# facebookresearch/co-tracker

Hardware: NVIDIA H100
Metric: tracked points*frames/sec at N=6400, T=16, 512^2 (higher is better)
Workload: dtype transformer + corr_mlp.fc2 + input_transform: bf16x3; correlation einsum: fp16x2; corr_mlp.fc1: bf16x3; fp32 accumulate, fp32 softmax/LayerNorm/GELU

## Files before the change

cotracker_b200/csrc/api_loop.cu:

```cuda
#include <math.h>

#include <string>
#include <vector>

#include "abi.cuh"

using namespace ct3;

namespace {

struct Block {
  Lin qkv_h;
  Lin q;
  Lin kv;
  Lin out, fc1, fc2;
  size_t ctx_g = 0, ctx_b = 0;
  bool cross = false;
};
struct Layout {
  Lin corr_fc1, corr_fc2, in_tr;
  Lin corr_fc1_h;
  Lin corr_fc1_t, corr_fc1_th;
  Block time[kDepth], vself[kDepth], p2v[kDepth], v2p[kDepth];
  size_t heads_w = 0, heads_b = 0, virt = 0, win_f32 = 0;
  size_t total = 0;
};

void place_block(Block& b, bool cross, size_t& off, bool time = false) {
  b.cross = cross;
  if (time) place_lin(b.qkv_h, 3 * kC, kC, off);
  if (cross) {
    b.ctx_g = off; off = align_up(off + kC * sizeof(float));
    b.ctx_b = off; off = align_up(off + kC * sizeof(float));
    place_lin(b.q, kC, kC, off);
    place_lin(b.kv, 2 * kC, kC, off);
  } else {
    place_lin(b.q, 3 * kC, kC, off);
  }
  place_lin(b.out, kC, kC, off);
  place_lin(b.fc1, kMlpHid, kC, off);
  place_lin(b.fc2, kC, kMlpHid, off);
}
const Layout& layout() {
  static const Layout L0 = [] {
    Layout L;
    size_t off = 0;
    place_lin(L.corr_fc1, kCorrHid, kVol, off);
    place_lin(L.corr_fc1_h, kCorrHid, kVol, off);
    place_lin(L.corr_fc1_t, kCorrHid, kVol, off);
    place_lin(L.corr_fc1_th, kCorrHid, kVol, off);
    place_lin(L.corr_fc2, kCorrOut, kCorrHid, off);
    place_lin(L.in_tr, kC, kX, off);
    L.win_f32 = off; off = align_up(off + (size_t)kC * kX * sizeof(float));
    L.virt = off;    off = align_up(off + (size_t)kV * kC * sizeof(float));
    L.heads_w = off; off = align_up(off + 4 * kC * sizeof(float));
    L.heads_b = off; off = align_up(off + 4 * sizeof(float));
    for (int i = 0; i < kDepth; ++i) {
      place_block(L.time[i], false, off,  true);
      place_block(L.vself[i], false, off);
      place_block(L.p2v[i], true, off);
      place_block(L.v2p[i], true, off);
    }
    L.total = off;
    return L;
  }();
  return L0;
}

const std::vector<std::string>& weight_names() {
  static const std::vector<std::string> names0 = [] {
    std::vector<std::string> names;
    const char* head[] = {"corr_mlp.fc1.weight", "corr_mlp.fc1.bias", "corr_mlp.fc2.weight", "corr_mlp.fc2.bias",
                          "updateformer.input_transform.weight", "updateformer.input_transform.bias",
                          "updateformer.virual_tracks", "updateformer.flow_head.weight", "updateformer.flow_head.bias",
                          "updateformer.vis_conf_head.weight", "updateformer.vis_conf_head.bias"};
    for (const char* h : head) names.push_back(h);
    const char* self_t[] = {"attn.to_q.weight", "attn.to_q.bias", "attn.to_kv.weight", "attn.to_kv.bias",
                            "attn.to_out.weight", "attn.to_out.bias", "mlp.fc1.weight", "mlp.fc1.bias",
                            "mlp.fc2.weight", "mlp.fc2.bias"};
    const char* cross_t[] = {"norm_context.weight", "norm_context.bias", "cross_attn.to_q.weight",
                             "cross_attn.to_q.bias", "cross_attn.to_kv.weight", "cross_attn.to_kv.bias",
                             "cross_attn.to_out.weight", "cross_attn.to_out.bias", "mlp.fc1.weight", "mlp.fc1.bias",
                             "mlp.fc2.weight", "mlp.fc2.bias"};
    for (int i = 0; i < kDepth; ++i) {
      const std::string idx = std::to_string(i) + ".";
      for (const char* t : self_t) names.push_back("updateformer.time_blocks." + idx + t);
      for (const char* t : self_t) names.push_back("updateformer.space_virtual_blocks." + idx + t);
      for (const char* t : cross_t) names.push_back("updateformer.space_point2virtual_blocks." + idx + t);
      for (const char* t : cross_t) names.push_back("updateformer.space_virtual2point_blocks." + idx + t);
    }
    return names;
  }();
  return names0;
}

struct Workspace {
  __nv_bfloat16* vol;
  __nv_bfloat16* h1;
  __nv_bfloat16* xs;
  float* tokens;
  __nv_bfloat16* ln;
  __nv_bfloat16* att;
  float* qkv;
  float* vqkv;
  __nv_bfloat16* hmid;
  float* row_bias;
  float* att_part;
  __nv_bfloat16* pyr_split;
  int32_t* groups;
  int32_t* frames;
  int32_t* track_len;
  int32_t* track_group;
  int slab;
  size_t total;
  bool slabbed() const { return slab_rows < point_rows; }
  int64_t slab_rows = 0, point_rows = 0;
};
int partial_slots(int N, int G) {
  if (G == 1) return kAttnMaxSplits;
  const int64_t s = kAttnMaxSplits + ((int64_t)N + 63LL * G) / 128;
  return (int)(s < (int64_t)kAttnMaxSplits * G ? s : (int64_t)kAttnMaxSplits * G);
}
int64_t group_table_ints(int N, int G) { return (int64_t)5 * G + 1 + 2 * ((int64_t)N / 128 + G); }
bool grouped(const ct3_loop_shape& s) { return s.G > 1 || s.group_T; }

Workspace carve(void* base, const ct3_loop_shape& s) {
  Workspace w;
  const int T = s.T, N = s.N, G = s.G, H4 = s.H4, W4 = s.W4, T_pyr = s.T_pyr > 0 ? s.T_pyr : s.T;
  w.slab = s.slab_tracks > 0 && s.slab_tracks < N ? s.slab_tracks : N;
  const size_t R = (size_t)(N + (size_t)kV * G) * T, Rp = (size_t)N * T, Rv = (size_t)kV * G * T;
  const size_t S = (size_t)w.slab * T, Mc = S * kL;
  w.slab_rows = (int64_t)S;
  w.point_rows = (int64_t)Rp;
  const bool sl = w.slabbed();
  Carver c(base);
  w.vol = (__nv_bfloat16*)c.take(Mc * 2 * kVolPad * 2);
  w.h1 = (__nv_bfloat16*)c.take(Mc * 2 * kCorrHid * 2);
  w.xs = (__nv_bfloat16*)c.take(S * 2 * kXPad * 2);
  w.tokens = (float*)c.take(R * kC * 4);
  w.ln = (__nv_bfloat16*)c.take((S + Rv) * 2 * kC * 2);
  w.att = (__nv_bfloat16*)c.take((S + Rv) * 2 * kC * 2);
  w.qkv = (float*)c.take(sl ? (S * 3 > Rp * 2 ? S * 3 : Rp * 2) * kC * 4 : R * 3 * kC * 4);
  w.vqkv = (float*)c.take(Rv * 3 * kC * 4);
  w.hmid = (__nv_bfloat16*)c.take((sl ? S : R) * 2 * kMlpHid * 2);
  w.row_bias = (float*)c.take((size_t)(s.group_T ? G : 1) * T * kC * 4);
  w.att_part = (float*)c.take(attention_partial_bytes(T, kV, partial_slots(N, G)));
  w.pyr_split = nullptr;
  if (H4 > 0 && W4 > 0 && corr_patch_supported(T_pyr, H4, W4))
    w.pyr_split = (__nv_bfloat16*)c.take((size_t)pyramid_layout(T_pyr, H4, W4).total * 4);
  w.groups = grouped(s) ? (int32_t*)c.take((size_t)group_table_ints(N, G) * 4) : nullptr;
  w.frames = s.T_pyr > 0 ? (int32_t*)c.take((size_t)G * T * 4) : nullptr;
  w.track_len = s.group_T ? (int32_t*)c.take(((size_t)N + (size_t)kV * G) * 4) : nullptr;
  w.track_group = s.group_T ? (int32_t*)c.take((size_t)N * 4) : nullptr;
  w.total = c.off;
  return w;
}

struct Runner {
  const uint8_t* pk;
  const Layout& L;
  cudaStream_t s;
  int impl;

  int gemm(const char* what, const __nv_bfloat16* x, const Lin& lin, int M, const GemmEpilogue& e, int products = 3,
           int fp16 = 0, int64_t x_ld = 0) {
    GemmProblem p;
    p.products = products;
    p.fp16 = fp16;
    p.x_ld = x_ld;
    p.x_split = x;
    p.w_split = reinterpret_cast<const __nv_bfloat16*>(pk + lin.w);
    p.M = M;
    p.N = lin.N;
    p.Kpad = lin.Kpad;
    p.epi = e;
    if (!p.epi.bias) p.epi.bias = reinterpret_cast<const float*>(pk + lin.b);
    if (M == 0) return 0;
    ProfScope ps(s, CAT_GEMM, 2.0 * (double)M * lin.N * lin.K);
    return run_gemm(p, impl, s, what);
  }
  static GemmEpilogue to_f32(float* out, int ld, bool residual) {
    GemmEpilogue e;
    e.out_f32 = out; e.ld_f32 = ld; e.residual = residual ? 1 : 0;
    return e;
  }
  static GemmEpilogue to_split(__nv_bfloat16* out, int ld, int lo_off, int act) {
    GemmEpilogue e;
    e.out_split = out; e.ld_split = ld; e.lo_off = lo_off; e.act = act;
    return e;
  }
};

#define RUNC(cat, call)                                        \
  do {                                                         \
    cudaError_t e__;                                           \
    { ProfScope ps__(R.s, cat); e__ = (cudaError_t)(call); }   \
    if (e__ != cudaSuccess) return fail_cuda(e__, #call);      \
  } while (0)
#define GEMM(...)                                                              \
  do {                                                                         \
    if (int rc__ = R.gemm("gemm(" #__VA_ARGS__ ")", __VA_ARGS__)) return rc__; \
  } while (0)

int run_attention(Runner& R, const Workspace& W, const AttnParams& a, bool per_warp) {
  if (g_opt_attn == 1) return (int)launch_attention(a, R.s);
  if (!per_warp && a.Lq > kV && attention_p2v_supported(a)) return (int)launch_attention_p2v(a, R.s);
  return (int)launch_attention_tc(a, per_warp, W.att_part, num_sms(), R.s);
}

AttnParams attn_params(const float* q, int q_ld, const float* kv, int kv_ld, int k_col, int v_col, __nv_bfloat16* out,
                       int Lq, int Lk, int T, int tracks = 0) {
  AttnParams a{};
  a.q = q; a.q_ld = q_ld; a.q_col = 0;
  a.kv = kv; a.kv_ld = kv_ld; a.k_col = k_col; a.v_col = v_col;
  a.out = out; a.out_ld = 2 * kC; a.lo_off = kC;
  a.num_seq = tracks ? tracks : T; a.Lq = Lq; a.Lk = Lk;
  a.q_seq_stride = a.k_seq_stride = tracks ? T : 1;
  a.q_tok_stride = a.k_tok_stride = tracks ? 1 : T;
  a.scale = 1.0f / sqrtf((float)kDh);
  return a;
}

struct GroupPlan {
  int G = 1, max_n = 0;
  const int32_t *off = nullptr, *all = nullptr, *split = nullptr, *slot = nullptr, *small = nullptr, *tile = nullptr;
  int n_small = 0, n_tiles = 0, split_max = 1, split_slots = 0;
  const int32_t *track_len = nullptr, *track_len_host = nullptr;
};

int plan_groups(GroupPlan& gp, const int32_t* sizes, int G, int T, int N, const int32_t* group_T, int32_t* dev,
                cudaStream_t s) {
  gp.G = G;
  if (G == 1 && !group_T) return 0;
  std::vector<int32_t> h((size_t)group_table_ints(N, G), 0);
  int32_t* off = h.data();
  int32_t *all = off + G + 1, *split = all + G, *slot = split + G, *small = slot + G, *tile = small + G;
  const int nsm = num_sms();
  for (int g = 0; g < G; ++g) {
    const int n = sizes ? sizes[g] : N;
    off[g + 1] = off[g] + n;
    if (n > gp.max_n) gp.max_n = n;
    all[g] = g;
    split[g] = attention_tc_splits(group_T ? group_T[g] : T, kV, n, nsm);
    if (split[g] > 1) {
      slot[g] = gp.split_slots;
      gp.split_slots += split[g];
      if (split[g] > gp.split_max) gp.split_max = split[g];
    }
    if (n > kV) {
      for (int n0 = off[g]; n0 < off[g + 1]; n0 += 128, ++gp.n_tiles) {
        tile[2 * gp.n_tiles] = g;
        tile[2 * gp.n_tiles + 1] = n0;
      }
    } else {
      small[gp.n_small++] = g;
    }
  }
  if (gp.split_slots > partial_slots(N, G)) return fail(CT3_EINVAL, "split-K partials exceed the workspace%s");
  CK(launch_upload_i32(dev, h.data(), (int)h.size(), s), "upload group table");
  gp.off = dev;
  gp.all = dev + (all - off);
  gp.split = dev + (split - off);
  gp.slot = dev + (slot - off);
  gp.small = dev + (small - off);
  gp.tile = dev + (tile - off);
  return 0;
}

int space_attention(Runner& R, const Workspace& W, const GroupPlan& gp, AttnParams a, bool q_pts, bool k_pts) {
  if (!gp.off) return run_attention(R, W, a, false);
  const int T = a.num_seq, n_all = a.Lq;
  a.goff = gp.off;
  a.frames = T;
  a.q_grp_stride = q_pts ? 0 : (int64_t)kV * a.q_tok_stride;
  a.k_grp_stride = k_pts ? 0 : (int64_t)kV * a.k_tok_stride;
  a.Lq = q_pts ? gp.max_n : kV;
  a.Lk = k_pts ? gp.max_n : kV;
  AttnParams b = a;
  b.gl = gp.all;
  b.num_seq = T * gp.G;
  if (g_opt_attn == 1) return (int)launch_attention(b, R.s);
  if (!q_pts) {
    if (k_pts) { b.gsplit = gp.split; b.gslot = gp.slot; b.split_max = gp.split_max; b.split_slots = gp.split_slots; }
    return (int)launch_attention_tc(b, false, W.att_part, num_sms(), R.s);
  }
  if (gp.n_small > 0) {
    b.gl = gp.small;
    b.num_seq = T * gp.n_small;
    b.Lq = kV;
    if (int rc = (int)launch_attention_tc(b, false, W.att_part, num_sms(), R.s)) return rc;
  }
  if (gp.n_tiles > 0) {
    AttnParams c = a;
    c.gtile = gp.tile;
    c.tiles = gp.n_tiles;
    c.Lq = n_all;
    c.Lk = kV * gp.G;
    return (int)launch_attention_p2v(c, R.s);
  }
  return 0;
}

int time_attention(Runner& R, const Workspace& W, const Block& b, const __nv_bfloat16* x, __nv_bfloat16* att,
                   int rows, int T, const int32_t* len = nullptr, const int32_t* len_host = nullptr) {
  const bool fuse = g_opt[OPT_FUSE] == 1 && R.impl == 0 && g_opt_attn != 1;
  auto fused = [&](int track0, int tracks) -> int {
    ProfScope ps(R.s, CAT_QKVA, 0.0);
    const char* gerr = nullptr;
    const int64_t r0 = (int64_t)track0 * T;
    const int rc = gemm_qkv_time_attn_launch(
        x + r0 * 2 * kC, reinterpret_cast<const __nv_bfloat16*>(R.pk + b.qkv_h.w),
        reinterpret_cast<const float*>(R.pk + b.qkv_h.b), tracks * T, kC, T, len ? len + track0 : nullptr,
        att + r0 * 2 * kC, 2 * kC, kC, 1.0f / sqrtf((float)kDh), num_sms(), R.s, &gerr);
    return rc ? fail_launch(rc, "fused qkv + time attention", gerr) : 0;
  };
  auto unfused = [&](int track0, int tracks) -> int {
    const int64_t r0 = (int64_t)track0 * T;
    GEMM(x + r0 * 2 * kC, b.q, tracks * T, Runner::to_f32(W.qkv, 3 * kC, false));
    AttnParams a = attn_params(W.qkv, 3 * kC, W.qkv, 3 * kC, kC, 2 * kC, att + r0 * 2 * kC, T, T, T, tracks);
    a.seq_len = len ? len + track0 : nullptr;
    RUNC(CAT_ATTN, run_attention(R, W, a, true));
    return 0;
  };
  if (fuse && qkv_time_attn_supported(T)) return fused(0, rows / T);
  if (!fuse || !len_host) return unfused(0, rows / T);
  for (int i = 0, n = rows / T; i < n;) {
    const bool short_run = qkv_time_attn_supported(len_host[i]);
    int j = i + 1;
    while (j < n && qkv_time_attn_supported(len_host[j]) == short_run) ++j;
    if (short_run) {
      if (int rc = fused(i, j - i)) return rc;
      const size_t row_bytes = 2 * kC * sizeof(__nv_bfloat16);
      CK(cudaMemset2DAsync(att + ((int64_t)i * T + 128) * 2 * kC, (size_t)T * row_bytes, 0,
                           (size_t)(T - 128) * row_bytes, (size_t)(j - i), R.s),
         "zero padded time-attention rows");
    } else if (int rc = unfused(i, j - i)) {
      return rc;
    }
    i = j;
  }
  return 0;
}

int64_t scratch_row(const Workspace& W, int64_t row, int64_t slab_row0) { return W.slabbed() ? row - slab_row0 : row; }

template <class F>
int for_slabs(const Workspace& W, int N, int n_begin, int n_end, F&& f) {
  if (!W.slabbed()) return f(n_begin, n_end - n_begin);
  for (int n = n_begin; n < n_end;) {
    const int stop = n < N && n_end > N ? N : n_end;
    const int count = stop - n < W.slab ? stop - n : W.slab;
    if (int rc = f(n, count)) return rc;
    n += count;
  }
  return 0;
}

int mlp_half(Runner& R, const Workspace& W, const Block& b, int64_t row0, int rows, int64_t slab_row0) {
  float* x = W.tokens + row0 * kC;
  const int64_t s = scratch_row(W, row0, slab_row0);
  __nv_bfloat16* ln = W.ln + s * 2 * kC;
  __nv_bfloat16* hm = W.hmid + s * 2 * kMlpHid;
  RUNC(CAT_LN, launch_layernorm_split(x, rows, nullptr, nullptr, 1e-6f, ln, R.s));
  GEMM(ln, b.fc1, rows, Runner::to_split(hm, 2 * kMlpHid, kMlpHid,  2));
  GEMM(hm, b.fc2, rows, Runner::to_f32(x, kC, true));
  return 0;
}

int transformer_body(Runner& R, const Workspace& W, int T, int N, const GroupPlan& gp) {
  const Layout& L = R.L;
  const int NV = kV * gp.G, Rp = N * T, Rv = NV * T;
  const uint8_t* pk = R.pk;
  RUNC(CAT_MISC, launch_init_virtual(W.tokens, reinterpret_cast<const float*>(pk + L.virt), T, N, gp.G, R.s));
  float* vtok = W.tokens + (int64_t)Rp * kC;
  __nv_bfloat16* ln_v = W.ln + W.slab_rows * 2 * kC;
  __nv_bfloat16* att_v = W.att + W.slab_rows * 2 * kC;
  float* q_p = W.qkv;
  __nv_bfloat16* att_p = W.slabbed() ? reinterpret_cast<__nv_bfloat16*>(W.qkv + (int64_t)Rp * kC) : W.att;
  auto ln_gemm_points = [&](const Block& b, bool ctx, const Lin& lin, float* out, int ld) {
    return for_slabs(W, N, 0, N, [&](int n, int count) -> int {
      const int64_t r0 = (int64_t)n * T;
      __nv_bfloat16* ln = W.ln + scratch_row(W, r0, r0) * 2 * kC;
      RUNC(CAT_LN, launch_layernorm_split(W.tokens + r0 * kC, count * T,
                                          ctx ? reinterpret_cast<const float*>(pk + b.ctx_g) : nullptr,
                                          ctx ? reinterpret_cast<const float*>(pk + b.ctx_b) : nullptr,
                                          ctx ? 1e-5f : 1e-6f, ln, R.s));
      GEMM(ln, lin, count * T, Runner::to_f32(out + r0 * ld, ld, false));
      return 0;
    });
  };
  auto mlp_tracks = [&](const Block& b, int n_begin, int n_end) {
    return for_slabs(W, N, n_begin, n_end, [&](int n, int count) -> int {
      return mlp_half(R, W, b, (int64_t)n * T, count * T, (int64_t)n * T);
    });
  };

  for (int i = 0; i < kDepth; ++i) {
    {
      const Block& b = L.time[i];
      if (int rc = for_slabs(W, N, 0, N + NV, [&](int n, int count) -> int {
            const int64_t r0 = (int64_t)n * T;
            const int rows = count * T;
            const int64_t s0 = scratch_row(W, r0, r0);
            float* x = W.tokens + r0 * kC;
            RUNC(CAT_LN, launch_layernorm_split(x, rows, nullptr, nullptr, 1e-6f, W.ln + s0 * 2 * kC, R.s));
            if (int rc = time_attention(R, W, b, W.ln + s0 * 2 * kC, W.att + s0 * 2 * kC, rows, T,
                                        gp.track_len ? gp.track_len + n : nullptr,
                                        gp.track_len_host ? gp.track_len_host + n : nullptr))
              return rc;
            GEMM(W.att + s0 * 2 * kC, b.out, rows, Runner::to_f32(x, kC, true));
            return mlp_half(R, W, b, r0, rows, r0);
          }))
        return rc;
    }
    {
      const Block& b = L.v2p[i];
      RUNC(CAT_LN, launch_layernorm_split(vtok, Rv, nullptr, nullptr, 1e-6f, ln_v, R.s));
      GEMM(ln_v, b.q, Rv, Runner::to_f32(W.vqkv, kC, false));
      if (int rc = ln_gemm_points(b, true, b.kv, W.qkv, 2 * kC)) return rc;
      RUNC(CAT_ATTN, space_attention(R, W, gp, attn_params(W.vqkv, kC, W.qkv, 2 * kC, 0, kC, att_v, kV, N, T), false,
                                     true));
      GEMM(att_v, b.out, Rv, Runner::to_f32(vtok, kC, true));
      if (int rc = mlp_tracks(b, N, N + NV)) return rc;
    }
    {
      const Block& b = L.vself[i];
      RUNC(CAT_LN, launch_layernorm_split(vtok, Rv, nullptr, nullptr, 1e-6f, ln_v, R.s));
      GEMM(ln_v, b.q, Rv, Runner::to_f32(W.vqkv, 3 * kC, false));
      RUNC(CAT_ATTN, space_attention(R, W, gp, attn_params(W.vqkv, 3 * kC, W.vqkv, 3 * kC, kC, 2 * kC, att_v, kV, kV,
                                                           T), false, false));
      GEMM(att_v, b.out, Rv, Runner::to_f32(vtok, kC, true));
      if (int rc = mlp_tracks(b, N, N + NV)) return rc;
    }
    {
      const Block& b = L.p2v[i];
      if (int rc = ln_gemm_points(b, false, b.q, q_p, kC)) return rc;
      RUNC(CAT_LN, launch_layernorm_split(vtok, Rv, reinterpret_cast<const float*>(pk + b.ctx_g),
                                 reinterpret_cast<const float*>(pk + b.ctx_b), 1e-5f, ln_v, R.s));
      GEMM(ln_v, b.kv, Rv, Runner::to_f32(W.vqkv, 2 * kC, false));
      RUNC(CAT_ATTN, space_attention(R, W, gp, attn_params(q_p, kC, W.vqkv, 2 * kC, 0, kC, att_p, N, kV, T), true,
                                     false));
      if (int rc = for_slabs(W, N, 0, N, [&](int n, int count) -> int {
            const int64_t r0 = (int64_t)n * T;
            GEMM(att_p + r0 * 2 * kC, b.out, count * T, Runner::to_f32(W.tokens + r0 * kC, kC, true));
            return mlp_half(R, W, b, r0, count * T, r0);
          }))
        return rc;
    }
  }
  return 0;
}

struct Prec {
  int corr, fc1; bool patch;
  bool vol16() const { return fc1 < 3; }
  bool support_major() const { return patch && corr != 3; }
};
Prec effective_prec(bool have_pyr_split, int T, int H4, int W4) {
  Prec p;
  p.patch = corr_uses_patch_kernel(g_opt_corr, have_pyr_split, T, H4, W4);
  p.corr = p.patch ? g_opt[OPT_PREC_CORR] : 3;
  p.fc1 = p.patch ? g_opt[OPT_PREC_FC1] : 3;
  return p;
}

int input_transform(Runner& R, const Workspace& W, int T, int n0, int count, const float* row_bias) {
  GemmEpilogue e = Runner::to_f32(W.tokens + (int64_t)n0 * T * kC, kC, false);
  if (row_bias) { e.row_bias = row_bias; e.row_mod = T; }
  if (row_bias && W.track_group) e.row_blk = W.track_group + n0;
  GEMM(W.xs, R.L.in_tr, count * T, e);
  return 0;
}

int point_tokens_slab(Runner& R, const Workspace& W, const Prec& pr, const float* pyr, const __nv_bfloat16* pyr_split,
                      int H4, int W4, const float* support, const uint8_t* track_valid, const float* coords,
                      const float* vis, const float* conf, int T, int N, int T_pyr, const FrameMap& fm, int n0,
                      int count) {
  const Layout& L = R.L;
  const int Mc = count * T * kL;
  RUNC(CAT_CORR, launch_corr_sample(pyr, pyr_split, H4, W4, support, track_valid, coords, T, N, n0, count, W.vol,
                                    g_opt_corr, pr.corr, pr.vol16() ? 1 : 0, num_sms(), R.s, T_pyr, fm));
  if (pr.vol16()) {
    GEMM(W.vol, pr.support_major() ? L.corr_fc1_th : L.corr_fc1_h, Mc,
         Runner::to_split(W.h1, 2 * kCorrHid, kCorrHid,  1), pr.fc1,  1, kVolPad);
  } else {
    GEMM(W.vol, pr.support_major() ? L.corr_fc1_t : L.corr_fc1, Mc,
         Runner::to_split(W.h1, 2 * kCorrHid, kCorrHid,  1));
  }
  {
    GemmEpilogue e = Runner::to_split(W.xs, 2 * kXPad, kXPad, 0);
    e.row_group = kL;
    GEMM(W.h1, L.corr_fc2, Mc, e);
  }
  RUNC(CAT_MISC, launch_build_x_small(coords, vis, conf, T, N, n0, count, W.track_len, W.xs, R.s));
  return input_transform(R, W, T, n0, count, W.row_bias);
}

int point_tokens(Runner& R, const Workspace& W, const Prec& pr, const float* pyr, const __nv_bfloat16* pyr_split,
                 int H4, int W4, const float* support, const uint8_t* track_valid, const float* coords,
                 const float* vis, const float* conf, int T, int N, int T_pyr, const FrameMap& fm) {
  return for_slabs(W, N, 0, N, [&](int n0, int count) -> int {
    return point_tokens_slab(R, W, pr, pyr, pyr_split, H4, W4, support, track_valid, coords, vis, conf, T, N, T_pyr,
                             fm, n0, count);
  });
}


int transform_and_heads(Runner& R, const Workspace& W, int T, int N, const GroupPlan& gp, float* coords, float* vis,
                        float* conf, float* delta) {
  const Layout& L = R.L;
  if (int rc = transformer_body(R, W, T, N, gp)) return rc;
  RUNC(CAT_MISC, launch_heads(W.tokens, reinterpret_cast<const float*>(R.pk + L.heads_w),
                              reinterpret_cast<const float*>(R.pk + L.heads_b), coords, vis, conf, delta, T, N, R.s));
  return 0;
}

int check_TN(int T, int N, int G = 1) {
  if (T < 1 || N < 1) return fail(CT3_EINVAL, "T and N must be >= 1%s");
  if (G < 1 || G > N) return fail(CT3_EINVAL, "G must be in [1, N]%s");
  if (((int64_t)N + (int64_t)kV * G) * T * 3 * kC >= (int64_t)1 << 40) return fail(CT3_EINVAL, "problem too large%s");
  return 0;
}

constexpr int64_t kSlabbedMaxRows = (int64_t)1 << 21;

enum class Use { kSize, kLoop, kFormer };

int check_shape(const ct3_loop_shape* sh, Use use) {
  if (!sh) return fail(CT3_EINVAL, "null shape%s");
  const ct3_loop_shape& s = *sh;
  if (int rc = check_TN(s.T, s.N, s.G)) return rc;
  if (s.group_T)
    for (int g = 0; g < s.G; ++g)
      if (s.group_T[g] < 1 || s.group_T[g] > s.T) return fail(CT3_EINVAL, "every group_T entry must be in [1, T]%s");
  if (s.group_sizes) {
    int64_t sum = 0;
    for (int g = 0; g < s.G; ++g) {
      if (s.group_sizes[g] < 1) return fail(CT3_EINVAL, "every group size must be >= 1%s");
      sum += s.group_sizes[g];
    }
    if (sum != s.N) return fail(CT3_EINVAL, "group sizes must sum to N%s");
  } else if (use != Use::kSize && s.G > 1) {
    return fail(CT3_EINVAL, "null group_sizes with G > 1%s");
  }
  if (s.slab_tracks < 0) return fail(CT3_EINVAL, "slab_tracks must be >= 0%s");
  if (s.slab_tracks > 0 && ((int64_t)s.N + (int64_t)kV * s.G) * s.T > kSlabbedMaxRows)
    return fail(CT3_EINVAL, "problem too large for track slabs: (N + 64 G) * T must be <= 2^21%s");
  if (s.T_pyr < 0 || (s.T_pyr == 0 && s.group_frames))
    return fail(CT3_EINVAL, "T_pyr must be >= 1 with a frame map and 0 without one%s");
  if (s.T_pyr > 0) {
    if (s.group_frames) {
      for (int64_t i = 0; i < (int64_t)s.G * s.T; ++i)
        if (s.group_frames[i] < 0 || s.group_frames[i] >= s.T_pyr)
          return fail(CT3_EINVAL, "frame index outside [0, T_pyr)%s");
    } else if (use != Use::kSize) {
      return fail(CT3_EINVAL, "null group_frames with T_pyr >= 1%s");
    }
  }
  const bool former = s.H4 == 0 && s.W4 == 0 && s.T_pyr == 0 && s.slab_tracks == 0;
  if (use == Use::kFormer || (use == Use::kSize && former)) return 0;
  const int T_pyr = s.T_pyr > 0 ? s.T_pyr : s.T;
  if ((int64_t)T_pyr * s.T >= (int64_t)1 << 31) return fail(CT3_EINVAL, "problem too large%s");
  return check_pyramid(T_pyr, s.H4, s.W4);
}

int update_loop(const void* packed, const float* pyr, const float* support, const uint8_t* track_valid, float* coords,
                float* vis, float* conf, const float* time_emb, int iters, const ct3_loop_shape* shape,
                void* workspace, size_t workspace_bytes, cudaStream_t stream) {
  if (!packed || !pyr || !support || !coords || !vis || !conf || !time_emb || !workspace)
    return fail(CT3_EINVAL, "null argument%s");
  if (int rc = check_shape(shape, Use::kLoop)) return rc;
  if (iters < 0) return fail(CT3_EINVAL, "iters must be >= 0%s");
  if (int rc = check_aligned(workspace, "workspace")) return rc;
  const ct3_loop_shape& s = *shape;
  const int T = s.T, N = s.N, G = s.G, H4 = s.H4, W4 = s.W4, T_pyr = s.T_pyr > 0 ? s.T_pyr : s.T;
  const Workspace W = carve(workspace, s);
  if (int rc = check_space(workspace_bytes, W.total, "workspace")) return rc;
  const Layout& L = layout();
  Runner R{reinterpret_cast<const uint8_t*>(packed), L, stream, g_opt_gemm};
  GroupPlan gp;
  if (int rc = plan_groups(gp, s.group_sizes, G, T, N, s.group_T, W.groups, R.s)) return rc;
  std::vector<int32_t> track_len;
  if (s.group_T) {
    track_len.resize((size_t)N + (size_t)kV * G);
    std::vector<int32_t> track_group((size_t)N);
    for (int g = 0, n0 = 0; g < G; ++g) {
      const int n = s.group_sizes ? s.group_sizes[g] : N;
      for (int i = 0; i < n; ++i) { track_len[n0 + i] = s.group_T[g]; track_group[n0 + i] = g; }
      for (int i = 0; i < kV; ++i) track_len[(size_t)N + (size_t)kV * g + i] = s.group_T[g];
      n0 += n;
    }
    CK(launch_upload_i32(W.track_len, track_len.data(), (int)track_len.size(), R.s), "upload track lengths");
    CK(launch_upload_i32(W.track_group, track_group.data(), N, R.s), "upload track groups");
    gp.track_len = W.track_len;
    gp.track_len_host = track_len.data();
  }
  FrameMap fm;
  if (s.T_pyr > 0) {
    CK(launch_upload_i32(W.frames, s.group_frames, G * T, R.s), "upload frame map");
    fm.frames = W.frames;
    fm.goff = G > 1 ? gp.off : nullptr;
// ... 356 lines not shown
```

cotracker_b200/csrc/attention_p2v.cu:

```cuda
#include "gemm.cuh"
#include "kernels.cuh"

namespace ct3 {
namespace {

constexpr int PV_THREADS = 128;
constexpr int PV_STQ = 128 * kDh * 4;
constexpr int PV_STK = 64 * kDh * 4;
constexpr int PV_TILE_Q = 128 * 128;
constexpr int PV_TILE_K = 64 * 128;
constexpr int PV_OFF_SQ = 0;
constexpr int PV_OFF_SK = PV_OFF_SQ + PV_STQ;
constexpr int PV_OFF_SV = PV_OFF_SK + PV_STK;
constexpr int PV_OFF_Q = PV_OFF_SV + PV_STK;
constexpr int PV_OFF_K = PV_OFF_Q + 2 * PV_TILE_Q;
constexpr int PV_OFF_V = PV_OFF_K + 2 * PV_TILE_K;
constexpr int PV_OFF_BAR = PV_OFF_V + kDh * 128;
constexpr int PV_OFF_END = PV_OFF_V + 2 * PV_TILE_K;
constexpr int PV_SMEM = PV_OFF_END + 1024;
constexpr uint32_t PV_LOAD_BYTES = PV_STQ + 2 * PV_STK;
static_assert(2 * (PV_SMEM + 1024) <= 233472, "two CTAs per SM");
static_assert(128 * kDh * 2 <= PV_TILE_Q, "one plane of output rows fits one Q/P tile");
static_assert(kDh == 48 && kV == 64, "chunk arithmetic below");

struct P2vMaps { CUtensorMap q, kv, out; };

__device__ __forceinline__ uint32_t swz(int r, int c16) { return (uint32_t)(r * 128 + ((c16 ^ (r & 7)) << 4)); }

__global__ void __launch_bounds__(PV_THREADS, 2)
attn_p2v_tc_kernel(const __grid_constant__ P2vMaps maps, AttnParams p, int tiles_per_seq) {
  extern __shared__ __align__(1024) uint8_t smem_raw[];
  uint8_t* smem = smem_align1024(smem_raw);
  uint64_t* bar_ld = reinterpret_cast<uint64_t*>(smem + PV_OFF_BAR);
  const int r = threadIdx.x, warp = r >> 5, lane = r & 31;
  const int t = blockIdx.x / tiles_per_seq, tile = blockIdx.x % tiles_per_seq;
  int n0 = tile * 128, kv0 = 0, n_end = p.Lq;
  if (p.gtile) {
    const int g = p.gtile[2 * tile];
    n0 = p.gtile[2 * tile + 1];
    kv0 = g * kV;
    n_end = p.goff[g + 1];
  }
  const bool tma_store = n0 + 128 <= n_end || n_end == p.Lq;

  for (int i = r; i < (PV_OFF_END - PV_OFF_Q) / 16; i += PV_THREADS)
    reinterpret_cast<uint4*>(smem + PV_OFF_Q)[i] = make_uint4(0, 0, 0, 0);
  __syncthreads();
  if (r == 0) {
    tma_prefetch_desc(&maps.q);
    tma_prefetch_desc(&maps.kv);
    tma_prefetch_desc(&maps.out);
    mbar_init(bar_ld, 1);
    fence_barrier_init();
  }
  __syncthreads();
  const float qscale = p.scale * 1.44269504088896340736f;
  const int rq = 16 * warp + (lane >> 2), cq = 2 * (lane & 3);
  const uint32_t sQ = smem_u32(smem + PV_OFF_Q), sK = smem_u32(smem + PV_OFF_K), sV = smem_u32(smem + PV_OFF_V);
  const int kv_key = (warp & 1) * 32 + lane, kv_c0 = (warp >> 1) * 6 + lane;

  auto issue_loads = [&](int h) {
    mbar_arrive_expect_tx(bar_ld, PV_LOAD_BYTES);
    tma_load_3d(smem + PV_OFF_SQ, &maps.q, p.q_col + h * kDh, t, n0, bar_ld);
    tma_load_3d(smem + PV_OFF_SK, &maps.kv, p.k_col + h * kDh, t, kv0, bar_ld);
    tma_load_3d(smem + PV_OFF_SV, &maps.kv, p.v_col + h * kDh, t, kv0, bar_ld);
  };
  if (r == 0) issue_loads(0);

  for (int h = 0; h < kHeads; ++h) {
    const uint32_t ph = (uint32_t)(h & 1);
    mbar_wait(bar_ld, ph);
    {
      const float4* sq = reinterpret_cast<const float4*>(smem + PV_OFF_SQ);
      const int slot = r & 7;
#pragma unroll
      for (int j = 0; j < 8; ++j) {
        const int row = j * 16 + (r >> 3);
        uint4 qh = make_uint4(0, 0, 0, 0), ql = make_uint4(0, 0, 0, 0);
        if (slot < 6) {
          const float4 a = sq[row * 12 + 2 * slot], b = sq[row * 12 + 2 * slot + 1];
          split2(a.x * qscale, a.y * qscale, qh.x, ql.x);
          split2(a.z * qscale, a.w * qscale, qh.y, ql.y);
          split2(b.x * qscale, b.y * qscale, qh.z, ql.z);
          split2(b.z * qscale, b.w * qscale, qh.w, ql.w);
        }
        *reinterpret_cast<uint4*>(smem + PV_OFF_Q + swz(row, slot)) = qh;
        *reinterpret_cast<uint4*>(smem + PV_OFF_Q + PV_TILE_Q + swz(row, slot)) = ql;
      }
      const float4* sk = reinterpret_cast<const float4*>(smem + PV_OFF_SK) + kv_key * 12;
      const float4* sv = reinterpret_cast<const float4*>(smem + PV_OFF_SV) + kv_key * 12;
#pragma unroll
      for (int j = 0; j < 6; ++j) {
        const int c = (kv_c0 + j) % 12;
        const float4 a = sk[c];
        uint32_t h0, l0, h1, l1;
        split2(a.x, a.y, h0, l0);
        split2(a.z, a.w, h1, l1);
        const uint32_t off = swz(kv_key, c >> 1) + (uint32_t)((c & 1) * 8);
        *reinterpret_cast<uint2*>(smem + PV_OFF_K + off) = make_uint2(h0, h1);
        *reinterpret_cast<uint2*>(smem + PV_OFF_K + PV_TILE_K + off) = make_uint2(l0, l1);
        const float4 b = sv[c];
        const float vals[4] = {b.x, b.y, b.z, b.w};
#pragma unroll
        for (int i = 0; i < 4; ++i) {
          const int d = 4 * c + i;
          const bf16pair sp = split_bf16(vals[i]);
          const uint32_t vo = swz(d, kv_key >> 3) + (uint32_t)((kv_key & 7) * 2);
          *reinterpret_cast<__nv_bfloat16*>(smem + PV_OFF_V + vo) = sp.hi;
          *reinterpret_cast<__nv_bfloat16*>(smem + PV_OFF_V + PV_TILE_K + vo) = sp.lo;
        }
      }
    }
    fence_proxy_async_smem();
    __syncthreads();
    if (r == 0 && h + 1 < kHeads) issue_loads(h + 1);
    float s0[32], s1[32];
    wgmma_fence();
#pragma unroll
    for (int kk = 0; kk < kDh / 16; ++kk) {
      const uint32_t ko = kk * 32;
      const uint64_t kh = gmma_desc_sw128(sK + ko), kl = gmma_desc_sw128(sK + PV_TILE_K + ko);
      const uint32_t first = kk != 0 ? 1u : 0u;
      wgmma_tile<64, false>(s0, gmma_desc_sw128(sQ + PV_TILE_Q + ko), kh, first);
      wgmma_tile<64, false>(s0, gmma_desc_sw128(sQ + ko), kl, 1u);
      wgmma_tile<64, false>(s0, gmma_desc_sw128(sQ + ko), kh, 1u);
      wgmma_tile<64, false>(s1, gmma_desc_sw128(sQ + 8192 + PV_TILE_Q + ko), kh, first);
      wgmma_tile<64, false>(s1, gmma_desc_sw128(sQ + 8192 + ko), kl, 1u);
      wgmma_tile<64, false>(s1, gmma_desc_sw128(sQ + 8192 + ko), kh, 1u);
    }
    wgmma_commit();
    wgmma_wait0(s0);
    wgmma_wait0(s1);
    __syncthreads();
#pragma unroll
    for (int hh = 0; hh < 2; ++hh) {
      float (&sc)[32] = hh ? s1 : s0;
#pragma unroll
      for (int rr = 0; rr < 2; ++rr) {
        float m = -INFINITY;
#pragma unroll
        for (int j = 0; j < 8; ++j) m = fmaxf(m, fmaxf(sc[4 * j + 2 * rr], sc[4 * j + 2 * rr + 1]));
        m = fmaxf(m, __shfl_xor_sync(0xffffffffu, m, 1));
        m = fmaxf(m, __shfl_xor_sync(0xffffffffu, m, 2));
        float l = 0.f;
#pragma unroll
        for (int j = 0; j < 8; ++j) {
          sc[4 * j + 2 * rr] = exp2f(sc[4 * j + 2 * rr] - m);
          sc[4 * j + 2 * rr + 1] = exp2f(sc[4 * j + 2 * rr + 1] - m);
          l += sc[4 * j + 2 * rr] + sc[4 * j + 2 * rr + 1];
        }
        l += __shfl_xor_sync(0xffffffffu, l, 1);
        l += __shfl_xor_sync(0xffffffffu, l, 2);
        const float inv = 1.0f / l;
        const int row = 64 * hh + rq + 8 * rr;
#pragma unroll
        for (int j = 0; j < 8; ++j) {
          uint32_t ph, pl;
          split2(sc[4 * j + 2 * rr] * inv, sc[4 * j + 2 * rr + 1] * inv, ph, pl);
          const uint32_t off = swz(row, j) + (uint32_t)(cq * 2);
          *reinterpret_cast<uint32_t*>(smem + PV_OFF_Q + off) = ph;
          *reinterpret_cast<uint32_t*>(smem + PV_OFF_Q + PV_TILE_Q + off) = pl;
        }
      }
    }
    fence_proxy_async_smem();
    __syncthreads();
    float o0[24], o1[24];
    wgmma_fence();
#pragma unroll
    for (int kk = 0; kk < 4; ++kk) {
      const uint32_t ko = kk * 32;
      const uint64_t vh = gmma_desc_sw128(sV + ko), vl = gmma_desc_sw128(sV + PV_TILE_K + ko);
      const uint32_t first = kk != 0 ? 1u : 0u;
      wgmma_tile<48, false>(o0, gmma_desc_sw128(sQ + PV_TILE_Q + ko), vh, first);
      wgmma_tile<48, false>(o0, gmma_desc_sw128(sQ + ko), vl, 1u);
      wgmma_tile<48, false>(o0, gmma_desc_sw128(sQ + ko), vh, 1u);
      wgmma_tile<48, false>(o1, gmma_desc_sw128(sQ + 8192 + PV_TILE_Q + ko), vh, first);
      wgmma_tile<48, false>(o1, gmma_desc_sw128(sQ + 8192 + ko), vl, 1u);
      wgmma_tile<48, false>(o1, gmma_desc_sw128(sQ + 8192 + ko), vh, 1u);
    }
    wgmma_commit();
    wgmma_wait0(o0);
    wgmma_wait0(o1);
    __syncthreads();
#pragma unroll
    for (int hh = 0; hh < 2; ++hh) {
      const float (&oc)[24] = hh ? o1 : o0;
#pragma unroll
      for (int rr = 0; rr < 2; ++rr) {
        const int row = 64 * hh + rq + 8 * rr;
#pragma unroll
        for (int j = 0; j < 6; ++j) {
          uint32_t oh, ol;
          split2(oc[4 * j + 2 * rr], oc[4 * j + 2 * rr + 1], oh, ol);
          const int off = row * (kDh * 2) + (8 * j + cq) * 2;
          *reinterpret_cast<uint32_t*>(smem + PV_OFF_Q + off) = oh;
          *reinterpret_cast<uint32_t*>(smem + PV_OFF_Q + PV_TILE_Q + off) = ol;
        }
      }
    }
    fence_proxy_async_smem();
    __syncthreads();
    if (tma_store) {
      if (r == 0) {
        tma_store_3d(&maps.out, h * kDh, t, n0, smem + PV_OFF_Q);
        tma_store_3d(&maps.out, p.lo_off + h * kDh, t, n0, smem + PV_OFF_Q + PV_TILE_Q);
        bulk_commit();
        bulk_wait_read0();
      }
    } else {
      for (int i = r; i < (n_end - n0) * 12; i += PV_THREADS) {
        const int row = i / 12, plane = (i % 12) / 6, c = i % 6;
        const uint4 v = *reinterpret_cast<const uint4*>(smem + PV_OFF_Q + plane * PV_TILE_Q + row * (kDh * 2) + c * 16);
        __nv_bfloat16* dst = p.out + ((int64_t)t * p.q_seq_stride + (int64_t)(n0 + row) * p.q_tok_stride) * p.out_ld +
                             plane * p.lo_off + h * kDh + c * 8;
        *reinterpret_cast<uint4*>(dst) = v;
      }
    }
    __syncthreads();
  }
  if (r == 0) bulk_wait0();
}

}

bool attention_p2v_supported(const AttnParams& p) {
  return (p.gtile ? p.Lk >= kV && p.Lk % kV == 0 : p.Lk == kV) && p.Lq >= 1 && (p.q_ld % 4) == 0 && (p.kv_ld % 4) == 0 && (p.q_col % 4) == 0 && (p.k_col % 4) == 0 &&
         (p.v_col % 4) == 0 && (p.out_ld % 8) == 0 && (p.lo_off % 8) == 0 &&
         ((reinterpret_cast<uintptr_t>(p.q) | reinterpret_cast<uintptr_t>(p.kv) | reinterpret_cast<uintptr_t>(p.out)) & 15) == 0;
}

cudaError_t launch_attention_p2v(const AttnParams& p, cudaStream_t s) {
  if (!attention_p2v_supported(p)) return cudaErrorInvalidValue;
  P2vMaps maps;
  {
    const uint64_t qd[3] = {(uint64_t)p.q_ld, (uint64_t)p.num_seq, (uint64_t)p.Lq};
    const uint64_t qs[2] = {(uint64_t)p.q_seq_stride * p.q_ld * 4, (uint64_t)p.q_tok_stride * p.q_ld * 4};
    const uint32_t qb[3] = {(uint32_t)kDh, 1, 128};
    const uint64_t kd[3] = {(uint64_t)p.kv_ld, (uint64_t)p.num_seq, (uint64_t)p.Lk};
    const uint64_t ks[2] = {(uint64_t)p.k_seq_stride * p.kv_ld * 4, (uint64_t)p.k_tok_stride * p.kv_ld * 4};
    const uint32_t kb[3] = {(uint32_t)kDh, 1, 64};
    const uint64_t od[3] = {(uint64_t)p.out_ld, (uint64_t)p.num_seq, (uint64_t)p.Lq};
    const uint64_t os[2] = {(uint64_t)p.q_seq_stride * p.out_ld * 2, (uint64_t)p.q_tok_stride * p.out_ld * 2};
    const uint32_t ob[3] = {(uint32_t)kDh, 1, 128};
    if (!encode_tensor_map(&maps.q, CU_TENSOR_MAP_DATA_TYPE_FLOAT32, 3, p.q, qd, qs, qb, CU_TENSOR_MAP_SWIZZLE_NONE) ||
        !encode_tensor_map(&maps.kv, CU_TENSOR_MAP_DATA_TYPE_FLOAT32, 3, p.kv, kd, ks, kb, CU_TENSOR_MAP_SWIZZLE_NONE) ||
        !encode_tensor_map(&maps.out, CU_TENSOR_MAP_DATA_TYPE_BFLOAT16, 3, p.out, od, os, ob, CU_TENSOR_MAP_SWIZZLE_NONE))
      return cudaErrorInvalidValue;
  }
  static DeviceOnce attr;
  cudaError_t e = once_per_device(attr, [&] {
    return cudaFuncSetAttribute(attn_p2v_tc_kernel, cudaFuncAttributeMaxDynamicSharedMemorySize, PV_SMEM);
  });
  if (e != cudaSuccess) return e;
  const int tiles = p.gtile ? p.tiles : (p.Lq + 127) / 128;
  attn_p2v_tc_kernel<<<p.num_seq * tiles, PV_THREADS, PV_SMEM, s>>>(maps, p, tiles);
  return cudaGetLastError();
}

}
```

cotracker_b200/csrc/kernels.cuh:

```cuda
#pragma once
#include "../../include/ct3_b200.h"
#include "common.cuh"

namespace ct3 {

struct PyramidLayout {
  int64_t off[kL];
  int h[kL], w[kL];
  int64_t total;
};
PyramidLayout pyramid_layout(int T, int H4, int W4);
cudaError_t launch_prepare_pyramid(const float* fmaps, int T, int H4, int W4, float* pyr, cudaStream_t s);
cudaError_t launch_sample_support(const float* pyr, int T, int H4, int W4, const int32_t* qframes,
                                  const float* qcoords, int N, const uint8_t* acc_mask, float* support,
                                  cudaStream_t s);

cudaError_t launch_pyramid_pools(int T, int H4, int W4, float* pyr, cudaStream_t s);

cudaError_t launch_prepare_frames(const void* src, int dtype, int T, int H, int W, int64_t st, int64_t sc, int64_t sh,
                                  int64_t sw, int oh, int ow, float* out, cudaStream_t s);

cudaError_t launch_finish_tracks(const float* fwd_tracks, const float* fwd_vis, const float* bwd_tracks,
                                 const float* bwd_vis, const float* queries, int B, int T, int N, int n_keep,
                                 float threshold, float scale_x, float scale_y, float* tracks, uint8_t* visibility,
                                 cudaStream_t s);

cudaError_t launch_online_window_begin(const ct3_online_stream* streams, int K, int64_t max_elems, int S, int step,
                                       float inv_stride, const int32_t* qframes, const float* qcoords, int N,
                                       uint8_t* valid, uint8_t* entering, int32_t* rel, float* coords_init,
                                       float* vis_init, float* conf_init, cudaStream_t s);
cudaError_t launch_online_window_end(const ct3_online_stream* streams, int K, int64_t max_elems, float stride,
                                     const float* coords, const float* vis, const float* conf, int N, float threshold,
                                     cudaStream_t s);

constexpr int kRenderMaxRadius = 255;
cudaError_t launch_render_prepare(const void* src, int dtype, int T, int H, int W, int64_t st, int64_t sc, int64_t sh,
                                  int64_t sw, int pad, int gray, uint8_t* out, cudaStream_t s);
cudaError_t launch_render_tracks(uint8_t* frames, int T, int H, int W, const float* pts, const uint8_t* visible,
                                 const uint8_t* colors, const uint8_t* draw_mask, int N, int radius, int linewidth,
                                 int trail, int query_frame, const double* alphas, const double* diff, int* keys,
                                 cudaStream_t s);
cudaError_t launch_render_flow_colors(const float* pts, int T, int N, int query_frame, uint8_t* colors, void* workspace,
                                      cudaStream_t s);

cudaError_t launch_im2col3x3_split(const float* in, int T, int C, int H, int W, int Kpad, __nv_bfloat16* out,
                                   cudaStream_t s);
size_t instnorm_scratch_bytes(int T, int C);
cudaError_t launch_instnorm_stats(const float* y, int T, int HW, int C, float eps, float* stats, void* scratch,
                                  cudaStream_t s);
cudaError_t launch_instnorm_relu_split(const float* y, const float* stats, int64_t rows, int HW, int C,
                                       __nv_bfloat16* out, cudaStream_t s);
cudaError_t launch_l2norm_rows(const float* in, int64_t rows, float* out, cudaStream_t s);
cudaError_t launch_upsample_concat(const float* const src[4], const int c[4], const int h[4], const int w[4], int T,
                                   int H, int W, float* out, cudaStream_t s);

cudaError_t launch_conv_stem(const float* frames, const float* w, const float* bias, int T, int H, int W, float* out,
                             cudaStream_t s);
cudaError_t launch_conv3x3_tc(const __nv_bfloat16* x_split, const __nv_bfloat16* w_split, const float* bias, int T,
                              int H, int W, int C, int Cout, float* out, int num_sms, cudaStream_t s);
cudaError_t launch_pack_conv(const float* w, int Cout, int Cin, int taps, int Cp, int Cout_pad, __nv_bfloat16* out,
                             cudaStream_t s);
cudaError_t launch_gather_s2(const __nv_bfloat16* x_split, int T, int H, int W, int C, int taps, __nv_bfloat16* out,
                             cudaStream_t s);
cudaError_t launch_norm_act(const float* y, const float* stats, const float* x, const float* stats_d, int mode,
                            int64_t rows, int HW, int C, float* out_f32, __nv_bfloat16* out_split, cudaStream_t s);
cudaError_t launch_upsample_concat_split(const float* const src[4], const int c[4], const int cs[4], const int h[4],
                                         const int w[4], int T, int Cp, int H, int W, __nv_bfloat16* out, cudaStream_t s);

struct FrameMap {
  const int32_t* frames = nullptr;
  const int32_t* goff = nullptr;
  int G = 1;
  int n0 = 0;
};
__device__ __forceinline__ const int32_t* frame_row(const FrameMap& m, int n, int T) {
  if (!m.frames) return nullptr;
  int g = 0;
  if (m.goff) {
    n += m.n0;
    int hi = m.G - 1;
    while (g < hi) {
      const int mid = (g + hi + 1) >> 1;
      if (__ldg(m.goff + mid) <= n) g = mid; else hi = mid - 1;
    }
  }
  return m.frames + (int64_t)g * T;
}
__device__ __forceinline__ int map_frame(const int32_t* row, int t) { return row ? __ldg(row + t) : t; }

bool corr_uses_patch_kernel(int impl, bool have_pyr_split, int T, int H4, int W4);
cudaError_t launch_corr_sample(const float* pyr, const __nv_bfloat16* pyr_split, int H4, int W4, const float* support,
                               const uint8_t* track_valid, const float* coords, int T, int N, int n0, int count,
                               __nv_bfloat16* vol_split, int impl, int mode, int vol16, int num_sms, cudaStream_t s,
                               int T_pyr, const FrameMap& fm);

cudaError_t launch_corr_sample_tc(const float* pyr, int H4, int W4, const float* support,
                                  const uint8_t* track_valid, const float* coords, int T, int N, int count,
                                  __nv_bfloat16* vol_split, int num_sms, cudaStream_t s, int T_pyr, const FrameMap& fm);

bool corr_patch_supported(int T, int H4, int W4);
cudaError_t launch_split_pyramid(const float* pyr, int T, int H4, int W4, __nv_bfloat16* pyr_split, int mode,
                                 cudaStream_t s);
cudaError_t launch_corr_patch_tc(const __nv_bfloat16* pyr_split, int H4, int W4, const float* support,
                                 const uint8_t* track_valid, const float* coords, int T, int N, int count,
                                 __nv_bfloat16* vol_split, int vol16, int num_sms, cudaStream_t s, int T_pyr,
                                 const FrameMap& fm);

cudaError_t launch_corr_patch_t(const __nv_bfloat16* pyr_half, int H4, int W4, const float* support,
                                const uint8_t* track_valid, const float* coords, int T, int N, int count,
                                __nv_bfloat16* vol, int vol16, int one_product, int num_sms, cudaStream_t s, int T_pyr,
                                const FrameMap& fm);

cudaError_t launch_layernorm_split(const float* x, int rows, const float* gamma, const float* beta, float eps,
                                   __nv_bfloat16* out_split, cudaStream_t s);
cudaError_t launch_build_x_small(const float* coords, const float* vis, const float* conf, int T, int N, int n0,
                                 int count, const int32_t* track_len, __nv_bfloat16* x_split, cudaStream_t s);
cudaError_t launch_init_virtual(float* tokens, const float* virt, int T, int N, int G, cudaStream_t s);
cudaError_t launch_upload_i32(int32_t* dst, const int32_t* src_host, int n, cudaStream_t s);
cudaError_t launch_heads(const float* tokens, const float* w4, const float* b4, float* coords, float* vis,
                         float* conf, float* delta_out, int T, int N, cudaStream_t s);
cudaError_t launch_row_bias(const float* time_emb, const float* w_in, int T, float* out, cudaStream_t s);
cudaError_t launch_split_rows(const float* x, int rows, int K, int Kpad, int perm_x, __nv_bfloat16* out,
                              int64_t dst_row_off, cudaStream_t s, int fp16 = 0);

struct AttnParams {
  const float* q;  int64_t q_ld;  int q_col;
  const float* kv; int64_t kv_ld; int k_col, v_col;
  __nv_bfloat16* out; int64_t out_ld; int lo_off;
  int num_seq, Lq, Lk;
  int64_t q_seq_stride, q_tok_stride;
  int64_t k_seq_stride, k_tok_stride;
  float scale;
  const int32_t* gl;
  const int32_t* goff;
  const int32_t* gsplit;
  const int32_t* gslot;
  int frames, split_max, split_slots;
  int64_t q_grp_stride, k_grp_stride;
  const int32_t* gtile;
  int tiles;
  const int32_t* seq_len;
};
struct SeqRows { int64_t q0, k0; int Lq, Lk, e, t; };
__device__ __forceinline__ SeqRows seq_rows(const AttnParams& p, int s) {
  SeqRows r;
  if (!p.gl) {
    r.q0 = (int64_t)s * p.q_seq_stride; r.k0 = (int64_t)s * p.k_seq_stride;
    r.Lq = p.Lq; r.Lk = p.seq_len ? p.seq_len[s] : p.Lk; r.e = 0; r.t = s;
    return r;
  }
  r.e = s / p.frames;
  r.t = s - r.e * p.frames;
  const int g = p.gl[r.e], n0 = p.goff[g], n = p.goff[g + 1] - n0;
  r.q0 = (int64_t)r.t * p.q_seq_stride + (p.q_grp_stride ? (int64_t)g * p.q_grp_stride : (int64_t)n0 * p.q_tok_stride);
  r.k0 = (int64_t)r.t * p.k_seq_stride + (p.k_grp_stride ? (int64_t)g * p.k_grp_stride : (int64_t)n0 * p.k_tok_stride);
  r.Lq = p.q_grp_stride ? kV : n;
  r.Lk = p.k_grp_stride ? kV : n;
  return r;
}
cudaError_t launch_attention(const AttnParams& p, cudaStream_t s);


constexpr int kAttnMaxSplits = 32;
size_t attention_partial_bytes(int num_seq, int Lq, int max_splits);
int attention_tc_splits(int num_seq, int Lq, int Lk, int num_sms);
cudaError_t launch_attention_tc(const AttnParams& p, bool per_warp, float* part, int num_sms, cudaStream_t s);

bool attention_p2v_supported(const AttnParams& p);
cudaError_t launch_attention_p2v(const AttnParams& p, cudaStream_t s);

}
```

Baseline: 646,500.

## Make point-to-virtual attention kernel persistent over (seq, tile, head) items

The p2v attention kernel used to launch one CTA per (sequence, 128-row tile) and loop over all heads inside it. It now launches a persistent grid of at most two CTAs per SM and strides over a flattened list of (sequence, tile, head) items, prefetching the next item's TMA loads while computing the current one. This aims to spread work more evenly across SMs and reduce tail effects and launch overhead. The cost is that Q is reloaded per head item, and the per-item tile lookups and store decision are recomputed on every iteration.

Result: no change. 647,300, median of 6 (+0.1%).

```diff
diff --git a/cotracker_b200/csrc/api_loop.cu b/cotracker_b200/csrc/api_loop.cu
--- a/cotracker_b200/csrc/api_loop.cu
+++ b/cotracker_b200/csrc/api_loop.cu
@@ -204,7 +204,7 @@
 
 int run_attention(Runner& R, const Workspace& W, const AttnParams& a, bool per_warp) {
   if (g_opt_attn == 1) return (int)launch_attention(a, R.s);
-  if (!per_warp && a.Lq > kV && attention_p2v_supported(a)) return (int)launch_attention_p2v(a, R.s);
+  if (!per_warp && a.Lq > kV && attention_p2v_supported(a)) return (int)launch_attention_p2v(a, num_sms(), R.s);
   return (int)launch_attention_tc(a, per_warp, W.att_part, num_sms(), R.s);
 }
 
@@ -296,7 +296,7 @@
     c.tiles = gp.n_tiles;
     c.Lq = n_all;
     c.Lk = kV * gp.G;
-    return (int)launch_attention_p2v(c, R.s);
+    return (int)launch_attention_p2v(c, num_sms(), R.s);
   }
   return 0;
 }
diff --git a/cotracker_b200/csrc/attention_p2v.cu b/cotracker_b200/csrc/attention_p2v.cu
--- a/cotracker_b200/csrc/attention_p2v.cu
+++ b/cotracker_b200/csrc/attention_p2v.cu
@@ -28,20 +28,26 @@
 __device__ __forceinline__ uint32_t swz(int r, int c16) { return (uint32_t)(r * 128 + ((c16 ^ (r & 7)) << 4)); }
 
 __global__ void __launch_bounds__(PV_THREADS, 2)
-attn_p2v_tc_kernel(const __grid_constant__ P2vMaps maps, AttnParams p, int tiles_per_seq) {
+attn_p2v_tc_kernel(const __grid_constant__ P2vMaps maps, AttnParams p, int tiles_per_seq, int items) {
   extern __shared__ __align__(1024) uint8_t smem_raw[];
   uint8_t* smem = smem_align1024(smem_raw);
   uint64_t* bar_ld = reinterpret_cast<uint64_t*>(smem + PV_OFF_BAR);
   const int r = threadIdx.x, warp = r >> 5, lane = r & 31;
-  const int t = blockIdx.x / tiles_per_seq, tile = blockIdx.x % tiles_per_seq;
-  int n0 = tile * 128, kv0 = 0, n_end = p.Lq;
-  if (p.gtile) {
-    const int g = p.gtile[2 * tile];
-    n0 = p.gtile[2 * tile + 1];
-    kv0 = g * kV;
-    n_end = p.goff[g + 1];
-  }
-  const bool tma_store = n0 + 128 <= n_end || n_end == p.Lq;
+  struct Item { int t, h, n0, kv0, n_end; };
+  auto item = [&](int i) {
+    Item it;
+    it.h = i % kHeads;
+    const int st = i / kHeads, tile = st % tiles_per_seq;
+    it.t = st / tiles_per_seq;
+    it.n0 = tile * 128; it.kv0 = 0; it.n_end = p.Lq;
+    if (p.gtile) {
+      const int g = p.gtile[2 * tile];
+      it.n0 = p.gtile[2 * tile + 1];
+      it.kv0 = g * kV;
+      it.n_end = p.goff[g + 1];
+    }
+    return it;
+  };
 
   for (int i = r; i < (PV_OFF_END - PV_OFF_Q) / 16; i += PV_THREADS)
     reinterpret_cast<uint4*>(smem + PV_OFF_Q)[i] = make_uint4(0, 0, 0, 0);
@@ -59,16 +65,19 @@
   const uint32_t sQ = smem_u32(smem + PV_OFF_Q), sK = smem_u32(smem + PV_OFF_K), sV = smem_u32(smem + PV_OFF_V);
   const int kv_key = (warp & 1) * 32 + lane, kv_c0 = (warp >> 1) * 6 + lane;
 
-  auto issue_loads = [&](int h) {
+  auto issue_loads = [&](const Item& it) {
     mbar_arrive_expect_tx(bar_ld, PV_LOAD_BYTES);
-    tma_load_3d(smem + PV_OFF_SQ, &maps.q, p.q_col + h * kDh, t, n0, bar_ld);
-    tma_load_3d(smem + PV_OFF_SK, &maps.kv, p.k_col + h * kDh, t, kv0, bar_ld);
-    tma_load_3d(smem + PV_OFF_SV, &maps.kv, p.v_col + h * kDh, t, kv0, bar_ld);
+    tma_load_3d(smem + PV_OFF_SQ, &maps.q, p.q_col + it.h * kDh, it.t, it.n0, bar_ld);
+    tma_load_3d(smem + PV_OFF_SK, &maps.kv, p.k_col + it.h * kDh, it.t, it.kv0, bar_ld);
+    tma_load_3d(smem + PV_OFF_SV, &maps.kv, p.v_col + it.h * kDh, it.t, it.kv0, bar_ld);
   };
-  if (r == 0) issue_loads(0);
-
-  for (int h = 0; h < kHeads; ++h) {
-    const uint32_t ph = (uint32_t)(h & 1);
+  if (r == 0 && (int)blockIdx.x < items) issue_loads(item(blockIdx.x));
+
+  uint32_t ph = 0;
+  for (int i = blockIdx.x; i < items; i += gridDim.x, ph ^= 1u) {
+    const Item it = item(i);
+    const int t = it.t, h = it.h, n0 = it.n0, n_end = it.n_end;
+    const bool tma_store = n0 + 128 <= n_end || n_end == p.Lq;
     mbar_wait(bar_ld, ph);
     {
       const float4* sq = reinterpret_cast<const float4*>(smem + PV_OFF_SQ);
@@ -113,7 +122,7 @@
     }
     fence_proxy_async_smem();
     __syncthreads();
-    if (r == 0 && h + 1 < kHeads) issue_loads(h + 1);
+    if (r == 0 && i + (int)gridDim.x < items) issue_loads(item(i + gridDim.x));
     float s0[32], s1[32];
     wgmma_fence();
 #pragma unroll
@@ -230,7 +239,7 @@
          ((reinterpret_cast<uintptr_t>(p.q) | reinterpret_cast<uintptr_t>(p.kv) | reinterpret_cast<uintptr_t>(p.out)) & 15) == 0;
 }
 
-cudaError_t launch_attention_p2v(const AttnParams& p, cudaStream_t s) {
+cudaError_t launch_attention_p2v(const AttnParams& p, int num_sms, cudaStream_t s) {
   if (!attention_p2v_supported(p)) return cudaErrorInvalidValue;
   P2vMaps maps;
   {
@@ -254,7 +263,9 @@
   });
   if (e != cudaSuccess) return e;
   const int tiles = p.gtile ? p.tiles : (p.Lq + 127) / 128;
-  attn_p2v_tc_kernel<<<p.num_seq * tiles, PV_THREADS, PV_SMEM, s>>>(maps, p, tiles);
+  const int items = p.num_seq * tiles * kHeads;
+  const int grid = items < 2 * num_sms ? items : 2 * num_sms;
+  attn_p2v_tc_kernel<<<grid, PV_THREADS, PV_SMEM, s>>>(maps, p, tiles, items);
   return cudaGetLastError();
 }
 
diff --git a/cotracker_b200/csrc/kernels.cuh b/cotracker_b200/csrc/kernels.cuh
--- a/cotracker_b200/csrc/kernels.cuh
+++ b/cotracker_b200/csrc/kernels.cuh
@@ -167,6 +167,6 @@
 cudaError_t launch_attention_tc(const AttnParams& p, bool per_warp, float* part, int num_sms, cudaStream_t s);
 
 bool attention_p2v_supported(const AttnParams& p);
-cudaError_t launch_attention_p2v(const AttnParams& p, cudaStream_t s);
+cudaError_t launch_attention_p2v(const AttnParams& p, int num_sms, cudaStream_t s);
 
 }
```
